# BradenDKelly/MetropolisMonteCarlo

Hardware: AMD Instinct MI355X
Metric: MC trial moves/sec (whole node), SPC/E NVT full Ewald fp64 (higher is better)
Workload: dtype f64

## Files before the change

metropolismontecarlo_amd/csrc/mmc_batch.inc:

```

#include <atomic>
#include <chrono>
#include <cmath>
#include <thread>
#include "mmc_state.hpp"
#include "mmc_solute_chain.hpp"

#define MMC_MAX_GROUPS 64
#define MMC_SERVER_AUTO_MAX 256
#define MMC_GEN_MAX 16
#define MMC_GEN_RING (MMC_GEN_MAX + 2)
#define MMC_QUEUE_STRIDE 32

#define MMC_CAND_EVERY 8
struct BatchCand {
    int enabled = 1;
    int skin_milli = 2000;
    bool tried = false;
    int state = 4;
    CandView v{};
    void *block = nullptr;
    int64_t bytes = 0;
    uint32_t t_build = 0;
    uint32_t d_refresh = 0;
    uint64_t epoch = ~0ULL;
    bool dirty = true;
    int64_t refresh_launches = 0;
    struct Range { int64_t r0, nr; unsigned long long count; bool pending; };
    std::vector<Range> ranges;
};

struct BatchSolute {
    int n = 0;
    bool charged = false;
    double mol[3 * (SOL_MAX_SITES + 1)] = { 0 };
    double charge[SOL_MAX_SITES] = { 0 }, eps[3 * SOL_MAX_SITES] = { 0 }, sig[3 * SOL_MAX_SITES] = { 0 };
    double q2 = 0.0;
    uint64_t hash = 0;
    double *d_par = nullptr;
    PartOut *h_parts = nullptr, *d_parts = nullptr;
    SoluteView view() const { return SoluteView{ d_par, n, charged ? 1 : 0 }; }
};

struct mmc_batch {
    DeviceSystem sys;
    BatchCand cand;
    BatchSolute sol;
    double lj_rcut = 0, qq_rcut = 0;
    int n_parts = 1;
    int kernel = 3;
    int server_wgs = -1;
    int wave_wgs = 0;
    int n_cus = 256;
    bool fast_ok = false;
    bool rigid_only = true;
    int image_by_molecule = -1;
    int zero_copy_moves = 0;
    MoveRec *h_moves[2] = { nullptr, nullptr };
    MoveRec *hd_moves[2] = { nullptr, nullptr };
    MoveRec *d_moves[2] = { nullptr, nullptr };
    PartOut *h_parts = nullptr, *d_parts = nullptr;
    int32_t *h_accept = nullptr, *d_accept = nullptr;
    int32_t *dev_accept = nullptr;
    int buf = 0;
    bool has_prev = false;
    std::vector<uint8_t> s_cur;
    std::vector<double> h_com, h_at;
    bool mirror_valid = false;
    int device_moves = 0;
    MoveRec *d_ring = nullptr;
    int ring_slots = MMC_GEN_RING;
    double *d_quat = nullptr;
    unsigned stamp = 0;
    int64_t steps_done = 0;
    int eval_parts = 0;
    int quat_mode = 0;
    double db[9] = { 0 };
    int persistent = -1;
    unsigned long long *h_ctrl = nullptr, *hd_ctrl = nullptr;
    unsigned long long *bar_ctrl = nullptr;
    int32_t *h_timeout = nullptr, *hd_timeout = nullptr;
    hipStream_t run_streams[MMC_MAX_GROUPS] = {};
    hipEvent_t run_events[MMC_MAX_GROUPS][2] = {};
    void *pool = nullptr;
    void (*pool_destroy)(void *) = nullptr;
    int steps_per_launch = 0;
    int whole_call = 0;
    int accept_on_device = -1;
    DecideConsts *d_decide = nullptr;
    DecideConsts decide_host{};
    std::vector<double> temps;
    double *d_temps = nullptr;
    unsigned *d_queue = nullptr;
    unsigned queue_base[MMC_MAX_GROUPS] = {};
    bool queue_reset = false;
    int server_stall_ms = 0;
    int64_t server_seq_offset = 0;
    bool needs_reload = false;
    std::vector<uint8_t> reloaded;
    int inject_torn = 0;
    bool vol_outstanding = false;
    bool vol_saved_fast_ok = false;
    int vol_saved_kernel = 0;
    std::vector<int32_t> pb_moved;
    int64_t trace_steps = 0;
    std::vector<double> trace_delta;
    std::vector<uint8_t> trace_flags;
    uint8_t *h_flags = nullptr, *hd_flags = nullptr, *d_flags = nullptr;
    uint8_t *bar_flags = nullptr;
    double2 *h_steps = nullptr, *hd_steps = nullptr, *d_steps = nullptr;
    void *obs_buf = nullptr;
    size_t obs_bytes = 0;
    void *obs_host = nullptr;
    size_t obs_host_bytes = 0;
    int coulomb_style = MMC_COULOMB_EWALD;
    bool s_stale = false;
    int local_stage = 1;
    int bond_chunk = 0;
    int ring_chunk = 0;
    int voronoi_prune = 1;
    uint64_t topology = 0;
    int state_chunk = 0;
    int state_delivery = -1;
    void *st_h[2] = { nullptr, nullptr }, *st_hd[2] = { nullptr, nullptr };
    void *st_d[2] = { nullptr, nullptr };
    size_t st_bytes = 0;
    hipEvent_t st_ev[2] = {};
    uint8_t *d_state_cur = nullptr;

// ... 515 lines not shown
                      b_cnt = up(2 * cqs * R), b_idx = up(2 * (int64_t)MMC_CAND_CAP * s.n_mol * R);
        const int64_t total = b_stat + b_d + b_q0 + b_cnt + b_idx;
        size_t free_b = 0, total_b = 0;
        void *blk = nullptr;
        if (hipMemGetInfo(&free_b, &total_b) == hipSuccess
            && (size_t)total + std::max<size_t>(total_b / 16, (size_t)1 << 30) <= free_b
            && hipMalloc(&blk, (size_t)total) == hipSuccess) {
            s.allocs.push_back(blk);
            char *p = (char *)blk;
            c.v.stat = (unsigned long long *)p; p += b_stat;
            c.v.D = (uint32_t *)p; p += b_d;
            c.v.q0 = (uint16_t *)p; p += b_q0;
            c.v.cnt = (uint16_t *)p; p += b_cnt;
            c.v.idx = (uint16_t *)p;
            c.block = blk;
            c.bytes = total;
            MMC_HIP(hipMemsetAsync(blk, 0, (size_t)(total - b_idx), s.stream));
            c.dirty = true;
        } else {
            (void)hipGetLastError();
            c.state = 2;
        }
    }
    if (!c.v.idx)
        return MMC_OK;
    const double gate_sq = std::max(pp.lj_gate_sq, pp.qq_gate_sq), gate = std::sqrt(gate_sq);
    const double wide = gate + 1e-3 * c.skin_milli;
    const uint32_t t_build = com_quant_gate(wide * wide, s.box);
    const uint32_t budget = cand_budget(t_build, com_quant_gate(gate_sq, s.box));
    if (t_build != c.t_build || budget != c.v.budget) {
        c.t_build = t_build;
        c.v.budget = budget;
        c.dirty = true;
    }
    c.d_refresh = (uint32_t)(((uint64_t)budget * 3 / 4) * ((uint64_t)budget * 3 / 4));
    c.state = budget > 0 ? 1 : 3;
    if (c.dirty || c.epoch != s.comq_epoch) {
        MMC_HIP(hipMemsetAsync(c.v.D, 0xff, sizeof(uint32_t) * (size_t)s.R, s.stream));
        MMC_HIP(hipStreamSynchronize(s.stream));
        c.dirty = false;
        c.epoch = s.comq_epoch;
        for (BatchCand::Range &g : c.ranges)
            g.pending = true;
    }
    return MMC_OK;
}

static int32_t batch_cand_stale(mmc_batch *b, hipStream_t stream, int64_t r0, int64_t nr)
{
    if (b->cand.v.idx) {
        MMC_HIP(hipMemsetAsync(b->cand.v.D + r0, 0xff, sizeof(uint32_t) * (size_t)nr, stream));
        for (BatchCand::Range &g : b->cand.ranges)
            if (g.r0 < r0 + nr && r0 < g.r0 + g.nr)
                g.pending = true;
    }
    return MMC_OK;
}

static int32_t batch_cand_for_launch(mmc_batch *b, hipStream_t stream, int64_t r0, int64_t nr, CandView *out)
{
    BatchCand &c = b->cand;
    *out = CandView{};
    if (!c.enabled || !c.v.idx || c.v.budget == 0)
        return batch_cand_stale(b, stream, r0, nr);
    BatchCand::Range *g = nullptr;
    for (BatchCand::Range &x : c.ranges)
        if (x.r0 == r0 && x.nr == nr)
            g = &x;
    if (!g) {
        c.ranges.push_back(BatchCand::Range{ r0, nr, 0ULL, true });
        g = &c.ranges.back();
    }
    if (g->pending || g->count % MMC_CAND_EVERY == 0) {
        k_cand_refresh<<<(unsigned)nr, 256, 0, stream>>>(b->sys.bv, c.v, (int)r0, c.t_build, c.d_refresh);
        MMC_HIP(hipGetLastError());
        c.refresh_launches++;
        g->pending = false;
    }
    g->count++;
    *out = c.v;
    return MMC_OK;
}

struct WaveForm { bool subst, img, multi, wolf, ladder; };

static int32_t batch_launch(mmc_batch *b, hipStream_t stream, int64_t r0, int64_t nr, int P, int kernel,
                            int buf, bool has_prev, const PairParams &pp,
                            hipEvent_t before_kernel = nullptr, const DevGen *dg = nullptr,
                            unsigned stamp = 0, const DevDecide *dd = nullptr)
{
    DeviceSystem &s = b->sys;
    const MoveRec *cur, *prev;
    const uint8_t *flagv = nullptr;
    if (dg) {
        flagv = b->hd_flags;
        const double2 *stp = b->hd_steps;
        if (!b->zero_copy_moves) {
            if (dd ? dd->fetch_flags : !b->bar_flags)
                k_fetch_bytes<<<(unsigned)((nr + 1023) / 1024), 256, 0, stream>>>(
                    b->d_flags + r0, b->hd_flags + r0, (int)nr);
            if (dg->upload_steps)
                MMC_HIP(hipMemcpyAsync(b->d_steps + r0, b->h_steps + r0, sizeof(double2) * nr,
                                       hipMemcpyHostToDevice, stream));
            flagv = b->bar_flags && !dd ? b->bar_flags : b->d_flags;
            stp = b->d_steps;
        }
        if (dg->n_gen > 0) {
            GenArgs ga;
            ga.steps = stp; ga.seed = dg->seed; ga.replica0 = dg->replica0;
            ga.rng_off = dg->rng_off; ga.step0 = dg->step; ga.n_gen = dg->n_gen;
            ga.ring = b->ring_slots; ga.ring_stride = s.R; ga.flag0 = flagv;
            ga.quat_mode = b->quat_mode;
            memcpy(ga.db, b->db, sizeof(ga.db));
            const int64_t n = nr * dg->n_gen;
            if (s.pb.on)
                k_propose<<<(unsigned)((n + 63) / 64), 64, 0, stream>>>(s.bv, s.rec, b->d_ring, ga, (int)r0,
                                                                        (int)nr, has_prev ? 1 : 0, s.pb_view());
            else
                k_propose<<<(unsigned)((n + 63) / 64), 64, 0, stream>>>(s.bv, s.rec, b->d_ring, ga,
                                                                        (int)r0, (int)nr, has_prev ? 1 : 0);
        }
        cur = batch_ring_slot(b, dg->step);
        prev = has_prev ? batch_ring_slot(b, dg->step + b->ring_slots - 1) : nullptr;
    } else {
        b->rigid_only = false;
        s.r_mol_max = INFINITY;
        if (!b->zero_copy_moves)
            MMC_HIP(hipMemcpyAsync(b->d_moves[buf] + r0, b->h_moves[buf] + r0,
                                   sizeof(MoveRec) * nr, hipMemcpyHostToDevice, stream));
        cur = b->dev_moves(buf);
        prev = has_prev ? b->dev_moves(buf ^ 1) : nullptr;
    }
    if (before_kernel)
        MMC_HIP(hipEventRecord(before_kernel, stream));
    if (b->sol.n)
        k_solute_move<<<(unsigned)((nr + SOLC_BLOCK / 16 - 1) / (SOLC_BLOCK / 16)), SOLC_BLOCK, 0, stream>>>(
            b->sol.view(), cur, s.qq_tab, s.fc, pp, s.box, b->sol.d_parts, (int)r0, (int)nr, stamp);
    dim3 grid((unsigned)P, (unsigned)nr);
    MMC_REQUIRE(!dd || (dg && P == 1 && !b->zero_copy_moves && kernel == 2), MMC_ERR_ASSERT,
                "the kernel's own accept decision needs device-side proposals, one part per move and the wave kernel");
    const bool wolf = b->coulomb_style == MMC_COULOMB_WOLF;
    if (kernel != 2)
        MMC_TRY(batch_cand_stale(b, stream, r0, nr));
    MMC_REQUIRE(!wolf || (kernel != 4 && !s.pb.on), MMC_ERR_ASSERT, "Wolf style reached a kernel without a Wolf form");
    using Yes = std::true_type;
    using No = std::false_type;
    if (kernel == 4) {
        MMC_REQUIRE(lat_applies(4 * P, (int)s.n_mol, (int)s.nkvecs), MMC_ERR_UNSUPPORTED,
                    "kernel 4 needs 4..%d parts (a multiple of 4) with at most %d molecules per pair "
                    "part", LAT_MAX_PARTS, LAT_MAXMOL);
        k_move_eval_lat<<<grid, LAT_WAVES * 64, 0, stream>>>(s.bv, s.rec, s.qq_tab, s.kpack, s.fc,
                                                             cur, prev, b->d_parts, 4 * P, pp, (int)r0,
                                                             flagv, stamp);
    } else if (kernel == 2) {
        const int64_t n_units = nr * P;
        int64_t wgs = (n_units + WV_MWAVES - 1) / WV_MWAVES;
        const int64_t cap = b->wave_wgs > 0 ? b->wave_wgs
                                            : (int64_t)(4 * (wolf ? WV_OCC_WOLF : WV_OCC) / WV_MWAVES) * b->n_cus;
        if (wgs > cap) wgs = cap;
        const bool img = dg && b->rigid_only && b->image_by_molecule != 0 &&
                         s.image_by_molecule(std::max(pp.lj_gate_sq, pp.qq_gate_sq)) &&
                         s.pairs_inside_slack(pp.qq_gate_sq, pp.qq_slack_sq) &&
                         s.pairs_inside_slack(pp.lj_gate_sq, pp.lj_slack_sq);
        const WaveForm f{ P != 1, img, dd && dd->n_sub > 1, wolf, dd && !b->temps.empty() };
        CandView cvv{};
        if (P == 1)
            MMC_TRY(batch_cand_for_launch(b, stream, r0, nr, &cvv));
        else
            MMC_TRY(batch_cand_stale(b, stream, r0, nr));
        auto launch = [&](auto subst, auto img_, auto multi, auto wolf_, auto ladder) {
            k_move_eval_wave<subst(), img_(), multi(), wolf_(), ladder()><<<(unsigned)wgs, WV_MWAVES * 64, 0, stream>>>(
                s.bv, s.rec, s.qq_tab, s.kpack, s.fc, cur, prev, dd ? dd->parts : b->d_parts, P, pp,
                (int)r0, (int)n_units, flagv, stamp, dd ? dd->dc : nullptr, dd ? (long long)dd->step : 0LL,
                dd ? dd->n_sub : 1, (int)(dg ? dg->step % b->ring_slots : 0), dd ? dd->queue : nullptr,
                dd ? dd->queue_base : 0u, cvv);
        };
        auto pick = [&](auto subst, auto img_, auto multi) {
            if (f.ladder) {
                if constexpr (!subst()) {
                    if (f.wolf) launch(subst, img_, multi, Yes{}, Yes{});
                    else launch(subst, img_, multi, No{}, Yes{});
                }
            } else if (f.wolf) launch(subst, img_, multi, Yes{}, No{});
            else launch(subst, img_, multi, No{}, No{});
        };
        if (f.multi) {
            if (f.img) pick(No{}, Yes{}, Yes{}); else pick(No{}, No{}, Yes{});
        } else if (!f.subst) {
            if (f.img) pick(No{}, Yes{}, No{}); else pick(No{}, No{}, No{});
        } else {
            if (f.img) pick(Yes{}, Yes{}, No{}); else pick(Yes{}, No{}, No{});
        }
    } else if (kernel == 1) {
        auto launch = [&](auto wolf_, const double *qq_tab, auto... per_box) {
            k_move_eval_fast<wolf_()><<<grid, MMC_BLOCK, 0, stream>>>(s.bv, s.rec, qq_tab, s.kpack, s.fc, cur, prev,
                                                                     b->d_parts, P, pp, (int)r0, flagv, stamp,
                                                                     per_box...);
        };
        if (s.pb.on) launch(No{}, nullptr, s.pb_view());
        else if (wolf) launch(Yes{}, s.qq_tab);
        else launch(No{}, s.qq_tab);
    } else {
        auto launch = [&](auto wolf_) {
            k_move_eval<wolf_()><<<grid, MMC_BLOCK, 0, stream>>>(s.bv, cur, prev, b->d_parts, P, pp, (int)r0,
                                                                 s.rec, flagv, stamp);
        };
        if (wolf) launch(Yes{}); else launch(No{});
    }
    MMC_HIP(hipGetLastError());
    return MMC_OK;
}

static int batch_server_parts(int64_t n_mol, int64_t R)
{
    int64_t pairs = (n_mol + 63) / 64;
    const int64_t cap = R == 1 ? 4 : SRV_WAVES - 1;
    if (pairs > cap) pairs = cap;
    if (pairs < 1) pairs = 1;
    return (int)pairs + 1;
}

static bool batch_server_applies(const mmc_batch *b)
{
    return b->fast_ok && b->kernel != 0 && b->device_moves && !b->quat_mode
           && b->sys.R <= (int64_t)b->n_cus;
}

static int batch_lat_shape(const mmc_batch *b)
{
    const DeviceSystem &s = b->sys;
    int G = b->server_wgs;
    if (G < 0)
        G = s.R * 4 <= (int64_t)b->n_cus ? 4 : 2;
    while (G >= 2 && !lat_applies(4 * G, (int)s.n_mol, (int)s.nkvecs))
        G--;
    if (G < 2 && b->server_wgs < 0) {
        G = (int)(((s.n_mol + LAT_MAXMOL - 1) / LAT_MAXMOL + 3 + LAT_WAVES - 1) / LAT_WAVES);
        while (G <= LAT_MAX_PARTS / LAT_WAVES && !lat_applies(4 * G, (int)s.n_mol, (int)s.nkvecs))
            G++;
        if (G > LAT_MAX_PARTS / LAT_WAVES)
            G = 0;
    }
    if (G < 2 || s.R * G > (int64_t)b->n_cus)
        return 0;
    return G;
}

static void batch_ctrl_clear(mmc_batch *b)
{
    memset(b->h_ctrl, 0, sizeof(unsigned long long) * b->sys.R);
    if (b->bar_ctrl) {
        for (int64_t r = 0; r < b->sys.R; r++)
            ((volatile unsigned long long *)b->bar_ctrl)[r] = 0ULL;
        mmc_bar_flush();
    }
}

static int32_t batch_server_start(mmc_batch *b, hipStream_t stream, int waves, const PairParams &pp,
// ... 443 lines not shown
```

metropolismontecarlo_amd/csrc/mmc_wave.hpp:

```cpp
#pragma once
#include "mmc_fast.hpp"
#include "mmc_propose.hpp"

#ifndef WV_WAVES
#define WV_WAVES 4
#endif
#ifndef WV_OCC
#define WV_OCC 5
#endif
#ifndef WV_OCC_WOLF
#define WV_OCC_WOLF 4
#endif
#ifndef WV_MWAVES
#define WV_MWAVES WV_WAVES
#endif
#ifndef WV_LIST
#define WV_LIST 640
#endif
#ifndef WV_PF
#define WV_PF 6
#endif
#define MMC_CQ_PAD (4 * 64 * (2 * WV_PF + 2))
#ifndef WV_TPF
#define WV_TPF 3
// ... 109 lines not shown
    return __builtin_amdgcn_readlane(v, src);
}

__device__ __forceinline__ double uniform_f64(double v)
{
    const long long b = __double_as_longlong(v);
    unsigned lo, hi;
    asm volatile("v_readfirstlane_b32 %0, %1" : "=s"(lo) : "v"((int)b));
    asm volatile("v_readfirstlane_b32 %0, %1" : "=s"(hi) : "v"((int)(b >> 32)));
    return __longlong_as_double((long long)(((unsigned long long)hi << 32) | lo));
}

__device__ __forceinline__ double lane_f64(double v, int src)
{
    const long long b = __double_as_longlong(v);
    const unsigned lo = (unsigned)__builtin_amdgcn_readlane((int)b, src);
    const unsigned hi = (unsigned)__builtin_amdgcn_readlane((int)(b >> 32), src);
    return __longlong_as_double((long long)(((unsigned long long)hi << 32) | lo));
}

__device__ __forceinline__ unsigned long long wave_shfl_xor_u64(unsigned long long v, int m)
{
    const unsigned lo = (unsigned)__shfl_xor((int)(unsigned)v, m, 64);
    const unsigned hi = (unsigned)__shfl_xor((int)(unsigned)(v >> 32), m, 64);
    return ((unsigned long long)hi << 32) | lo;
}
__device__ __forceinline__ unsigned long long wave_min_u64(unsigned long long v)
{
#pragma unroll
    for (int m = 32; m > 0; m >>= 1) {
        const unsigned long long o = wave_shfl_xor_u64(v, m);
        v = o < v ? o : v;
    }
    return v;
}

__device__ __forceinline__ void phase_row_moderate(double x, double L, cplx *row )
{
    double sn, cs;
    sincos_moderate(MMC_TWOPI * x / L, sn, cs);
    const cplx e1 = { cs, sn }, one = { 1.0, 0.0 };
    row[5] = one;
    row[6] = e1;
    row[4] = c_conj(e1);
    cplx p = e1;
#pragma unroll
    for (int k = 2; k <= 5; k++) {
        p = c_mul(p, e1);
        row[5 + k] = p;
        row[5 - k] = c_conj(p);
    }
}

template <bool LADDER = false>
__device__ __forceinline__ int wave_decide(const double *outw, bool ov_old, bool ov_new,
                                           const DecideConsts *__restrict__ dc, long long step, int r,
                                           int scur, int lane, double *delta_out = nullptr, bool store_flags = true,
                                           bool flip_s = true)
{
    const double delta = mmc_move_delta(outw, ov_old, ov_new, dc->factor);
    if (delta_out)
        *delta_out = delta;
    const double x = delta / (LADDER ? dc->temps[r] : dc->temperature);
    const double u = mmc_metropolis_uniform(ChainKey{ dc->seed, dc->replica0 + (uint32_t)r }, (uint64_t)step);
    bool met;
    if (x < 0.0) met = true;
    else if (1.0 - x > u + 1e-9) met = true;
    else if ((1.0 + x) * u > 1.0 + 1e-9) met = false;
    else met = exp(-x) > u;
    const int acc = (met && !(ov_old || ov_new)) ? 1 : 0;
    if (store_flags && lane == 0)
        dc->flags[r] = (uint8_t)(acc | ((scur ^ (flip_s ? acc : 0)) << 1));
    return acc;
}

__device__ __forceinline__ int wave_ticket(unsigned *queue, unsigned base, int n_waves, int lane)
{
    unsigned t = 0;
    if (lane == 0)
        t = atomicAdd(queue, 1u);
    return n_waves + (int)(__builtin_amdgcn_readfirstlane(t) - base);
}

template <bool SUBST, bool IMG, bool MULTI = false, bool WOLF = false, bool LADDER = false>
__global__ __launch_bounds__(WV_MWAVES * 64)
__attribute__((amdgpu_waves_per_eu(WOLF ? WV_OCC_WOLF : WV_OCC, WOLF ? WV_OCC_WOLF : WV_OCC))) void k_move_eval_wave(
    BatchView bv, double *rec, const double *__restrict__ qq_tab,
    const int32_t *__restrict__ kpack, FastConsts fc, const MoveRec *__restrict__ cur,
    const MoveRec *__restrict__ prev, PartOut *out, int n_parts, PairParams pp, int r_base,
    int n_units, const uint8_t *flagv, unsigned stamp, const DecideConsts *__restrict__ dc, long long dec_step,
    int n_sub_arg, int slot0, unsigned *queue, unsigned queue_base, CandView cv)
{
    const int n_sub = MULTI ? n_sub_arg : 1;
    const bool cand_on = !SUBST && cv.idx != nullptr;
    __shared__ __align__(16) WaveSharedT<WV_MWAVES, !WOLF> sm;
    const int tid = threadIdx.x, lane0 = tid & 63;
    const int wv = __builtin_amdgcn_readfirstlane(tid >> 6);

    for (int k = tid; k < MMC_QQ_TABLE_DOUBLES; k += WV_MWAVES * 64)
        sm.qtab[k] = qq_tab[k];
    __syncthreads();

    const int n_mol = bv.n_mol, nkv = bv.nkvecs;
    const double box = bv.box;
    const BoxConsts bc = box_consts(box);
    const int np = WOLF ? n_parts : (n_parts == 1) ? 1 : n_parts - 1;
    const int plen = (n_mol + np - 1) / np;
    const bool same_gate = pp.lj_gate_sq == pp.qq_gate_sq;
    const double inv_box = uniform_f64(1.0 / box);
    uint32_t gate_q;
    asm volatile("v_readfirstlane_b32 %0, %1" : "=s"(gate_q) : "v"(com_quant_gate(fmax(pp.lj_gate_sq, pp.qq_gate_sq), box)));
    wv_list_t *const list = sm.list[wv];
    const double *const pvw = sm.pvw[wv];

    for (int unit = blockIdx.x * WV_MWAVES + wv; unit < n_units;
         unit = MULTI && queue ? wave_ticket(queue, queue_base, gridDim.x * WV_MWAVES, lane0)
                               : unit + gridDim.x * WV_MWAVES) {
        int lane = lane0;
        if (!MULTI)
            asm volatile("" : "+v"(lane));
        int rl = unit, part = 0;
        if (n_parts != 1) {
            rl = unit / n_parts;
            part = unit - rl * n_parts;
        }
        const int r = r_base + rl;
        const bool do_pairs = WOLF ? true : (n_parts == 1) || (part < n_parts - 1);
        const bool do_recip = WOLF ? false : (n_parts == 1) || (part == n_parts - 1);
        const int j_begin = do_pairs ? min(part * plen, n_mol) : 0;
        const int j_end = do_pairs ? min(j_begin + plen, n_mol) : 0;
        double *const myrec = rec + (int64_t)r * n_mol * MMC_RSTRIDE;

        int flags_carry = -1;
        double e_sum = 0.0;
        unsigned acc_mask = 0, ovl_mask = 0, kind_mask = 0;
        uint32_t d_cur = MMC_CAND_STALE;
        unsigned n_cand = 0;
        if (!SUBST && cand_on)
            d_cur = (uint32_t)__builtin_amdgcn_readfirstlane((int)cv.D[r]);
      for (int sub = 0; sub < n_sub; sub++) {
        if (MULTI) {
            lane = lane0;
            asm volatile("" : "+v"(lane));
        }
        const MoveRec *cur_s = cur, *prev_s = prev;
        if (n_sub > 1) {
            const int sl = (slot0 + sub) % dc->ring_slots, slp = (slot0 + sub + dc->ring_slots - 1) % dc->ring_slots;
            cur_s = dc->ring + (int64_t)sl * dc->ring_stride;
            if (sub > 0)
                prev_s = dc->ring + (int64_t)slp * dc->ring_stride;
        }
        WV_STAMP(0);
        const double *mvp = reinterpret_cast<const double *>(cur_s + r);
        double w = 0.0;
        if (lane < MV_Q_NEW)
            w = mvp[lane];
        WV_STAMP(1);
        const int gflag = flags_carry >= 0 ? flags_carry : (flagv ? __builtin_amdgcn_readfirstlane((int)flagv[r]) : -1);
        const long long hdr = __double_as_longlong(w);
        const int i0 = lane_i32((int)hdr, 0) - 1;
        const int flags = gflag >= 0 ? gflag : lane_i32((int)(hdr >> 32), 0);
        const bool commit = prev_s && (flags & 1);
        const int scur = (flags >> 1) & 1;

        int pend = -1;
        uint32_t pcxy = 0, pcz = 0;
        if (commit) {
            const double *pvp = reinterpret_cast<const double *>(prev_s + r);
            double pw = 0.0;
            if (lane < 9) pw = pvp[MV_AT_NEW + lane];
            else if (lane < 12) pw = pvp[MV_COM_NEW + lane - 9];
            else if (lane == 12) pw = pvp[0];
            else if (lane < 17) pw = pvp[MV_Q_NEW + lane - 13];
            pend = lane_i32((int)__double_as_longlong(pw), 12) - 1;
            if (lane < 12)
                sm.pvw[wv][lane] = pw;
            if (part == 0 && lane < 12) {
                myrec[(int64_t)pend * MMC_RSTRIDE + lane] = pw;
                if (lane < 9) {
                    const int a = lane / 3, d = lane % 3;
                    (d == 0 ? bv.ax : d == 1 ? bv.ay : bv.az)[r * bv.atom_stride + 3 * pend + a] = pw;
                } else {
                    const int d = lane - 9;
                    (d == 0 ? bv.comx : d == 1 ? bv.comy : bv.comz)[r * bv.mol_stride + pend] = pw;
                    comq_store(bv, r, pend, d, pw, inv_box);
                }
            }
            if (!SUBST && cand_on) {
                const int cq = (lane >= 9 && lane < 12) ? (int)com_quant(pw, inv_box) : 0;
                pcxy = (uint32_t)lane_i32(cq, 9) | (uint32_t)lane_i32(cq, 10) << 16;
                pcz = (uint32_t)lane_i32(cq, 11);
            }
            if (bv.quat) {
                const double q0 = wave_pick(pw, 13), q1 = wave_pick(pw, 14),
                             q2 = wave_pick(pw, 15), q3 = wave_pick(pw, 16);
                if (part == 0 && lane >= 13 && lane < 17)
                    quat_commit(bv, r, pend, lane - 13, pw, q0 * q0 + q1 * q1 + q2 * q2 + q3 * q3 > 0.25);
            }
            wave_sync();
            if (WOLF && !SUBST)
                asm volatile("s_waitcnt vmcnt(0)" ::: "memory");
        }

#define WV_CQ_BASE (bv.comq + (int64_t)r * 3 * bv.cq_stride)
#define WV_PART_DST (out + (int64_t)r * n_parts + part)
        auto decide_here = [&](bool o0, bool o1) -> int {
            if (!dc)
                return 0;
            if (n_sub <= 1)
                return wave_decide<LADDER>(sm.outw[wv], o0, o1, dc, dec_step, r, scur, lane, nullptr, true, !WOLF);
            double delta;
            const bool last = sub + 1 == n_sub;
            const int acc = wave_decide<LADDER>(sm.outw[wv], o0, o1, dc, dec_step + sub, r, scur, lane, &delta, last, !WOLF);
            if (acc) {
                e_sum += delta;
                acc_mask |= 1u << sub;
            }
            if (o0 || o1)
                ovl_mask |= 1u << sub;
            kind_mask |= (unsigned)((lane_i32((int)(hdr >> 32), 0) >> 8) & 1) << sub;
            flags_carry = acc | ((scur ^ (WOLF ? 0 : acc)) << 1);
            if (last) {
                wave_sync();
                if (lane < 7)
                    sm.outw[wv][lane] = lane == 0 ? e_sum
                                 : lane == 1 ? __longlong_as_double((long long)acc_mask | ((long long)ovl_mask << 32))
                                 : lane == 2 ? __longlong_as_double((long long)kind_mask) : 0.0;
                wave_sync();
            }
            return acc;
        };
#define WV_DECIDE(o0, o1) decide_here(o0, o1)
#define WV_RECORD_OVL(o) (n_sub > 1 ? false : (o))
#define WV_STORE_IF (sub + 1 == n_sub)
#define WV_STORE_SYSTEM MULTI
#define WV_ZERO opaque_f64(0.0)
#define WV_SUBST SUBST
#define WV_IMG IMG
#define WV_WOLF WOLF
#define WV_VIRIAL (!MULTI)
#ifndef WV_XY_MOVE
#define WV_XY_MOVE 1
#endif
#define WV_XY WV_XY_MOVE
#define WV_PASSES 2
#ifndef WV_ONE_CALL_MOVE
#define WV_ONE_CALL_MOVE 1
#endif
#define WV_ONE_CALL WV_ONE_CALL_MOVE
#define WV_CAND (!SUBST)
#define WV_AFTER_PHASE_TABLES                                                                    \
    if (!SUBST && commit)                                                                        \
        asm volatile("s_waitcnt vmcnt(0)" ::: "memory");
#include "mmc_wave_unit.inc"
#undef WV_AFTER_PHASE_TABLES
#undef WV_IMG
#undef WV_WOLF
#undef WV_VIRIAL
#undef WV_PASSES
#undef WV_ONE_CALL
#undef WV_CAND
#undef WV_XY
#undef WV_SUBST
#undef WV_ZERO
#undef WV_CQ_BASE
#undef WV_PART_DST
#undef WV_DECIDE
#undef WV_RECORD_OVL
#undef WV_STORE_IF
#undef WV_STORE_SYSTEM
        if (n_sub > 1)
            asm volatile("s_waitcnt vmcnt(0)" ::: "memory");
      }
        if (!SUBST && cand_on && lane == 0) {
            atomicAdd(cv.stat + (int64_t)r * MMC_CAND_STATS, (unsigned long long)n_cand);
            atomicAdd(cv.stat + (int64_t)r * MMC_CAND_STATS + 1, (unsigned long long)((unsigned)n_sub - n_cand));
        }
    }
}

struct TotalWaveShared {
    alignas(16) double qtab[MMC_QQ_TABLE_DOUBLES];
    int32_t list[WV_WAVES][WV_LIST];
};

#define WV_TOTAL_WAVES_PER_SIMD 5
template <bool COHERENT, bool IMG>
__device__ __forceinline__ void total_wave_body(
    TotalWaveShared &sm, const BatchView &bv, const double *__restrict__ rec,
    const double *__restrict__ qq_tab, const FastConsts &fc, const PairParams &pp, TotalPart *out,
    int units_per_rep, int n_units, int paired, int wg, int n_wgs, int j_chunk = 0)
{
    const int tid = threadIdx.x, lane0 = tid & 63;
    const int wv = __builtin_amdgcn_readfirstlane(tid >> 6);
    for (int k = tid; k < MMC_QQ_TABLE_DOUBLES; k += WV_WAVES * 64)
        sm.qtab[k] = qq_tab[k];
    __syncthreads();

    const int n_mol = bv.n_mol;
    const double box = bv.box;
    const BoxConsts bc = box_consts(box);
    const bool same_gate = pp.lj_gate_sq == pp.qq_gate_sq;
    const double inv_box = 1.0 / box;
    const uint32_t gate_q = com_quant_gate(fmax(pp.lj_gate_sq, pp.qq_gate_sq), box);
    int32_t *const list = sm.list[wv];

    for (int unit = wg * WV_WAVES + wv; unit < n_units; unit += n_wgs * WV_WAVES) {
        int lane = lane0;
        asm volatile("" : "+v"(lane));
        const int r = unit / units_per_rep, u = unit - r * units_per_rep;
        const double *myrec = rec + (int64_t)r * n_mol * MMC_RSTRIDE;
        const uint16_t *cq0 = bv.comq + (int64_t)r * 3 * bv.cq_stride;
        const uint32_t *sxy = reinterpret_cast<const uint32_t *>(cq0);
        const uint16_t *sz = cq0 + 2 * bv.cq_stride;
        double a_lj = 0, a_v = 0, a_q = 0;
        unsigned long long ovm = 0;

        const int n_ch = j_chunk > 0 ? (n_mol + j_chunk - 1) / j_chunk : 1;
        const int j_lo = j_chunk > 0 ? (u % n_ch) * j_chunk : 0;
        const int j_hi = j_chunk > 0 ? min(j_lo + j_chunk, n_mol) : n_mol;
        const int iA = j_chunk > 0 ? u / n_ch : u, iB = n_mol - 1 - u;
        const bool hasB = paired && iB > iA;
        double wAB = 0.0;
        if (lane < MMC_REC)
            wAB = myrec[(int64_t)iA * MMC_RSTRIDE + lane];
        else if (hasB && lane >= 16 && lane < 16 + MMC_REC)
            wAB = myrec[(int64_t)iB * MMC_RSTRIDE + lane - 16];

        auto process = [&](int cnt) {
            wave_sync();
            for (int n0 = 0; n0 < cnt; n0 += 64) {
                const int n = n0 + lane;
                const bool act = n < cnt;
                const int ent = act ? list[n] : 0;
                const int j = ent & ((1 << 27) - 1);
                const bool isB = (ent >> 27) != 0;
                double t[MMC_REC];
                const double2 *src = reinterpret_cast<const double2 *>(myrec + (int64_t)j * MMC_RSTRIDE);
#pragma unroll
                for (int q = 0; q < 6; q++) {
                    const double2 v = src[q];
                    t[2 * q] = v.x;
                    t[2 * q + 1] = v.y;
                }
                const int own0 = isB ? 16 : 0;
                auto mine = [&](int word) { return wave_pick(wAB, own0 + word); };
                const double ccx = mine(9), ccy = mine(10), ccz = mine(11);
                double m[3] = { 0, 0, 0 };
                auto min1 = [&](int d, double a, double b) {
                    if constexpr (IMG)
                        return fma(m[d], bc.neg, b - a);
                    else
                        return vector1D_abs(a, b, bc);
                };
                if constexpr (IMG) {
                    const double dx = t[9] - ccx, dy = t[10] - ccy, dz = t[11] - ccz;
                    m[0] = (fabs(dx) < bc.half) ? 0.0 : copysign(1.0, dx);
// ... 364 lines not shown
```

metropolismontecarlo_amd/csrc/mmc_wave_unit.inc:

```
#ifndef WV_NS
#define WV_NS 2
#define WV_NS_DEFAULTED
#endif
#if WV_NS == 2
#define WV_IF2(...) __VA_ARGS__
#else
#define WV_IF2(...)
#endif
#ifndef WV_SUBST
#define WV_SUBST 1
#define WV_SUBST_DEFAULTED
#endif
#ifndef WV_IMG
#define WV_IMG 0
#define WV_IMG_DEFAULTED
#endif
#ifndef WV_PASSES
#define WV_PASSES 1
#define WV_PASSES_DEFAULTED
#endif
#ifndef WV_ONE_CALL
#define WV_ONE_CALL 0
#define WV_ONE_CALL_DEFAULTED
#endif
#ifndef WV_XY
#define WV_XY 0
#define WV_XY_DEFAULTED
#endif
#ifndef WV_KPF
#define WV_KPF 2
#endif
#ifndef WV_WOLF
#define WV_WOLF 0
#define WV_WOLF_DEFAULTED
#endif
#ifndef WV_ZERO
#define WV_ZERO 0.0
#define WV_ZERO_DEFAULTED
#endif
#ifndef WV_VIRIAL
#define WV_VIRIAL 1
#define WV_VIRIAL_DEFAULTED
#endif
#ifndef WV_STORE_IF
#define WV_STORE_IF true
#define WV_STORE_IF_DEFAULTED
#endif
#if WV_NS != 2
static_assert(WV_VIRIAL, "the one-state body always delivers the virial");
#endif
        double *const outw = sm.outw[wv];
        unsigned long long ovm0 = 0, ovm1 = 0;

        constexpr bool wv_wolf = WV_WOLF;
        if constexpr (!wv_wolf) {
        if (do_recip) {
            {
                const int t = lane < 18 ? lane : 0;
                const int st = t / 9, q = t - 9 * st;
                const double x = wave_pick(w, (st ? MV_AT_NEW : MV_AT_OLD) + q);
                if (lane < 18)
                    phase_row_moderate(x, box, sm.ptab[wv][st][q / 3][q % 3]);
            }
            wave_sync();
            WV_STAMP(2);
#ifdef WV_AFTER_PHASE_TABLES
            WV_AFTER_PHASE_TABLES
#endif
        }
        auto recip_loop = [&]() {
            double a_rec = 0;
#ifdef WV_S_BASE
            const double *So = WV_S_BASE;
            double *Sn = WV_S_DST;
#else
            const double *So = s_buf(bv, r, scur);
            double *Sn = s_buf(bv, r, scur ^ 1);
#endif
            int kcs[WV_KPF], kps[WV_KPF];
            double cfs[WV_KPF];
            double2 sos[WV_KPF];
#pragma unroll
            for (int q = 0; q < WV_KPF; q++) {
                kcs[q] = min(lane + 64 * q, nkv - 1);
                kps[q] = kpack[kcs[q]];
                cfs[q] = bv.cfac[kcs[q]];
                sos[q] = *reinterpret_cast<const double2 *>(So + 2 * kcs[q]);
            }
#if WV_XY
            const int colp = kpack[MMC_NK_STRIDE + lane];
#endif
#if WV_XY
            cplx xyp[2][3];
            {
                const int cx = colp & 15, cy = (colp >> 4) & 15;
#pragma unroll
                for (int st = 0; st < 2; st++)
#pragma unroll
                    for (int l = 0; l < 3; l++)
                        xyp[st][l] = c_mul_fused(sm.ptab[wv][st][l][0][5 + cx], sm.ptab[wv][st][l][1][cy]);
            }
#endif
#ifdef WV_S_MIRROR
            unsigned long long s_sum = 0;
#endif
            const int n_it = (nkv + 63) >> 6;
            int k = lane;
            for (int it = 0; it < n_it; it++) {
                const int kc = kcs[0], kp = kps[0];
                const double cf = cfs[0];
                const double2 so = sos[0];
#pragma unroll
                for (int q = 0; q + 1 < WV_KPF; q++) {
                    kcs[q] = kcs[q + 1]; kps[q] = kps[q + 1]; cfs[q] = cfs[q + 1]; sos[q] = sos[q + 1];
                }
                kcs[WV_KPF - 1] = min(k + 64 * WV_KPF, nkv - 1);
                kps[WV_KPF - 1] = kpack[kcs[WV_KPF - 1]];
                cfs[WV_KPF - 1] = bv.cfac[kcs[WV_KPF - 1]];
                sos[WV_KPF - 1] = *reinterpret_cast<const double2 *>(So + 2 * kcs[WV_KPF - 1]);
                {
                    const int kz = (kp >> 8) & 15;
                    double nr = so.x, ni = so.y;
#if WV_XY
                    const int col = (kp >> 12) & (MMC_KCOLS - 1);
                    auto from_col = [&](const cplx &v) {
                        cplx o;
                        o.re = wave_pick(v.re, col);
                        o.im = wave_pick(v.im, col);
                        return o;
                    };
#else
                    const int kx = kp & 15, ky = (kp >> 4) & 15;
#endif
#pragma unroll
                    for (int l = 0; l < 3; l++) {
#if WV_XY
                        const cplx tn = c_mul_fused(from_col(xyp[1][l]), sm.ptab[wv][1][l][2][kz]);
                        const cplx to = c_mul_fused(from_col(xyp[0][l]), sm.ptab[wv][0][l][2][kz]);
#else
                        const cplx tn = c_mul_fused(c_mul_fused(sm.ptab[wv][1][l][0][5 + kx], sm.ptab[wv][1][l][1][ky]),
                                                sm.ptab[wv][1][l][2][kz]);
                        const cplx to = c_mul_fused(c_mul_fused(sm.ptab[wv][0][l][0][5 + kx], sm.ptab[wv][0][l][1][ky]),
                                                sm.ptab[wv][0][l][2][kz]);
#endif
                        nr = fma(fc.q[l], tn.re - to.re, nr);
                        ni = fma(fc.q[l], tn.im - to.im, ni);
                    }
                    *reinterpret_cast<double2 *>(Sn + 2 * kc) = make_double2(nr, ni);
#ifdef WV_S_MIRROR
                    {
                        typedef double s_piece __attribute__((ext_vector_type(2)));
                        s_piece v;
                        v.x = nr; v.y = ni;
                        double *mp = WV_S_MIRROR + 2 * kc;
                        asm volatile("global_store_dwordx4 %0, %1, off sc0 sc1" ::"v"(mp), "v"(v) : "memory");
                        if (k < nkv)
                            s_sum += (unsigned long long)__double_as_longlong(nr)
                                     + 3ULL * (unsigned long long)__double_as_longlong(ni);
                    }
#endif
                    const double wgt = k < nkv ? cf : 0.0;
                    a_rec = fma(wgt, fma(nr, nr, ni * ni) - fma(so.x, so.x, so.y * so.y), a_rec);
                }
                k += 64;
            }
            wave_sum1_store(a_rec, &outw[6], outw, lane);
#ifdef WV_S_MIRROR
            s_sum = wave_sum_u64(s_sum);
            if (lane == 0)
                sm.pvw[wv][0] = __longlong_as_double((long long)s_sum);
#endif
            WV_STAMP(3);
            wave_sync();
        };
        if (do_recip)
            recip_loop();
        }
        if (!do_recip && lane == 0)
            outw[6] = WV_ZERO;

        if (do_pairs) {
            if (lane < 6)
                outw[lane] = WV_ZERO;
            double cc[2][3];
            uint32_t cqxy[2], cqz[2];
            {
                const bool is_com = WV_IF2((lane >= MV_COM_OLD && lane < MV_COM_OLD + 3) ||)
                                    (lane >= MV_COM_NEW && lane < MV_COM_NEW + 3);
                const int myq = is_com ? (int)com_quant(w, inv_box) : 0;
#pragma unroll
                for (int d = 0; d < 3; d++) {
                    WV_IF2(cc[0][d] = lane_f64(w, MV_COM_OLD + d);)
                    cc[1][d] = lane_f64(w, MV_COM_NEW + d);
                }
                WV_IF2(cqxy[0] = (uint32_t)lane_i32(myq, MV_COM_OLD) | (uint32_t)lane_i32(myq, MV_COM_OLD + 1) << 16;)
                cqxy[1] = (uint32_t)lane_i32(myq, MV_COM_NEW) | (uint32_t)lane_i32(myq, MV_COM_NEW + 1) << 16;
                WV_IF2(cqz[0] = (uint32_t)lane_i32(myq, MV_COM_OLD + 2);)
                cqz[1] = (uint32_t)lane_i32(myq, MV_COM_NEW + 2);
            }

            auto process = [&](int cnt) {
                WV_IF2(double a_lj0 = 0, a_v0 = 0, a_q0 = 0;)
                double a_lj1 = 0, a_v1 = 0, a_q1 = 0;
                wave_sync();
                for (int n0 = 0; n0 < cnt; n0 += 64) {
                    const int n = n0 + lane;
                    const int j = n < cnt ? list[n] : 0;
                    const bool act = (n < cnt) && (j != i0);
                    double t[MMC_REC];
                    const double2 *src = reinterpret_cast<const double2 *>(myrec + (int64_t)j * MMC_RSTRIDE);
#pragma unroll
                    for (int q = 0; q < 6; q++) {
                        const double2 v = src[q];
                        t[2 * q] = v.x;
                        t[2 * q + 1] = v.y;
                    }
                    if (n0 == 0)
                        WV_STAMP(5);
                    if (WV_SUBST && j == pend) {
#pragma unroll
                        for (int q = 0; q < MMC_REC; q++)
                            t[q] = pvw[q];
                    }
                    WV_IF2(bool g0, l0;)
                    bool g1, l1;
                    constexpr bool wv_img = WV_IMG;
                    constexpr bool wv_virial = WV_VIRIAL;
                    double m[2][3] = { { 0, 0, 0 }, { 0, 0, 0 } };
                    auto min1 = [&](int st, int d, double a, double b) {
                        if constexpr (wv_img)
                            return fma(m[st][d], bc.neg, b - a);
                        else
                            return vector1D_abs(a, b, bc);
                    };
#define WV_MIN1(st, d, a, b) min1(st, d, a, b)
                    {
                        if constexpr (wv_img) {
#pragma unroll
                            for (int d = 0; d < 3; d++) {
                                const double d1 = t[9 + d] - cc[1][d];
                                m[1][d] = (fabs(d1) < bc.half) ? 0.0 : copysign(1.0, d1);
#if WV_NS == 2
                                const double d0 = t[9 + d] - cc[0][d];
                                m[0][d] = (fabs(d0) < bc.half) ? 0.0 : copysign(1.0, d0);
#endif
                            }
                        }
#if WV_NS == 2
                        const double x0 = WV_MIN1(0, 0, cc[0][0], t[9]), y0 = WV_MIN1(0, 1, cc[0][1], t[10]),
                                     z0 = WV_MIN1(0, 2, cc[0][2], t[11]);
                        const double c0 = x0 * x0 + y0 * y0 + z0 * z0;
                        g0 = act && (c0 < pp.qq_gate_sq);
                        l0 = same_gate ? g0 : (act && (c0 < pp.lj_gate_sq));
#endif
                        const double x1 = WV_MIN1(1, 0, cc[1][0], t[9]), y1 = WV_MIN1(1, 1, cc[1][1], t[10]),
                                     z1 = WV_MIN1(1, 2, cc[1][2], t[11]);
                        const double c1 = x1 * x1 + y1 * y1 + z1 * z1;
                        g1 = act && (c1 < pp.qq_gate_sq);
                        l1 = same_gate ? g1 : (act && (c1 < pp.lj_gate_sq));
                    }
                    WV_IF2(const unsigned long long gm0 = wave_ballot(g0);)
                    const unsigned long long gm1 = wave_ballot(g1);
#if WV_PASSES == 2
#define WV_PAIR_FENCE
                    auto pass = [&](auto stc, bool l, unsigned long long gm, unsigned long long &ovm,
                                    double &a_lj, double &a_v, double &a_q) {
                        constexpr int ST = decltype(stc)::value;
                        auto atoms = [&](auto exc, uint32_t &umin) {
                        constexpr bool EXACT = decltype(exc)::value;
#pragma unroll 1
                        for (int a = 0; a < 3; a++) {
                            const int base_w = (ST ? MV_AT_NEW : MV_AT_OLD) + 3 * a;
                            const double ax = lane_f64(w, base_w), ay = lane_f64(w, base_w + 1),
                                         az = lane_f64(w, base_w + 2);
                            auto pair1 = [&](int ab, double bx, double by, double bz) {
                                const double qq = fc.qq9[ab];
                                const double px = WV_MIN1(ST, 0, ax, bx), py = WV_MIN1(ST, 1, ay, by),
                                             pz = WV_MIN1(ST, 2, az, bz);
                                const double u = px * px + py * py + pz * pz;
                                const unsigned long long km = (wv_img ? ~0ULL : wave_ballot(u < pp.qq_slack_sq)) & gm;
                                if constexpr (EXACT) {
                                    const bool qneg = (fc.qneg_mask >> ab) & 1;
                                    const unsigned long long cm = wave_ballot(u < pp.ovr) & gm;
                                    const unsigned long long qm = qneg ? cm : 0ULL, cold = cm & ~qm;
// ... 256 lines not shown
                        list[cnt + lanes_below(m)] = j;
                    cnt += __popcll(m & m_end);
                    base += 64;
                }
                pxy += 256 * WV_PF;
                pz += 128 * WV_PF;
#if WV_ONE_CALL
            }
#ifdef WV_CAND
            }
            cand_pre = false;
#endif
            WV_STAMP(4);
            if (cnt)
                process(cnt);
            }
#else
                if (cnt > WV_LIST - 64 * WV_PF) {
                    process(cnt);
                    cnt = 0;
                }
            }
            WV_STAMP(4);
            if (cnt)
                process(cnt);
#endif
            WV_STAMP(6);
        } else if (lane < 6) {
            outw[lane] = WV_ZERO;
        }
#ifdef WV_S_MIRROR
        if (do_recip && !do_pairs) {
            wave_sync();
            if (lane == 0)
                outw[0] = sm.pvw[wv][0];
        }
#endif

#ifdef WV_UNIT_NO_STORE
        if (lane == 0)
            outw[7] = __longlong_as_double((long long)((ovm0 != 0ULL ? 1 : 0) | (ovm1 != 0ULL ? 2 : 0)));
#else
        wave_sync();
        {
#ifdef WV_DECIDE
            const int accept = WV_DECIDE(ovm0 != 0ULL, ovm1 != 0ULL);
#else
            const int accept = 0;
#endif
            if (WV_STORE_IF) {
                const uint32_t csum = part_checksum_lanes(lane < 7 ? outw[lane] : 0.0, lane, stamp);
#ifdef WV_RECORD_OVL
                if (lane == 0)
                    outw[7] = pack_ovl(WV_RECORD_OVL(ovm0 != 0ULL), WV_RECORD_OVL(ovm1 != 0ULL), stamp, csum, accept);
#else
                if (lane == 0)
                    outw[7] = pack_ovl(ovm0 != 0ULL, ovm1 != 0ULL, stamp, csum, accept);
#endif
            }
        }
        wave_sync();
#ifdef WV_STORE_WT
        store_part<true>(WV_PART_DST, sm.outw[wv], lane);
#else
#ifndef WV_STORE_SYSTEM
#define WV_STORE_SYSTEM false
#define WV_STORE_SYSTEM_DEFAULTED
#endif
        if (WV_STORE_IF)
            store_part<WV_STORE_SYSTEM>(WV_PART_DST, sm.outw[wv], lane);
#ifdef WV_STORE_SYSTEM_DEFAULTED
#undef WV_STORE_SYSTEM
#undef WV_STORE_SYSTEM_DEFAULTED
#endif
#endif
        wave_sync();
        WV_STAMP(7);
#endif
#ifdef WV_STORE_IF_DEFAULTED
#undef WV_STORE_IF
#undef WV_STORE_IF_DEFAULTED
#endif
#undef WV_IF2
#ifdef WV_XY_DEFAULTED
#undef WV_XY
#undef WV_XY_DEFAULTED
#endif
#ifdef WV_ONE_CALL_DEFAULTED
#undef WV_ONE_CALL
#undef WV_ONE_CALL_DEFAULTED
#endif
#ifdef WV_PASSES_DEFAULTED
#undef WV_PASSES
#undef WV_PASSES_DEFAULTED
#endif
#ifdef WV_IMG_DEFAULTED
#undef WV_IMG
#undef WV_IMG_DEFAULTED
#endif
#ifdef WV_SUBST_DEFAULTED
#undef WV_SUBST
#undef WV_SUBST_DEFAULTED
#endif
#ifdef WV_ZERO_DEFAULTED
#undef WV_ZERO
#undef WV_ZERO_DEFAULTED
#endif
#ifdef WV_VIRIAL_DEFAULTED
#undef WV_VIRIAL
#undef WV_VIRIAL_DEFAULTED
#endif
#ifdef WV_WOLF_DEFAULTED
#undef WV_WOLF
#undef WV_WOLF_DEFAULTED
#endif
#ifdef WV_NS_DEFAULTED
#undef WV_NS
#undef WV_NS_DEFAULTED
#endif
```

Before: 157.3 million.

## Pass wave kernel arguments via cached device struct and reload per phase

Packs the wave kernel's large by-value arguments (BatchView, PairParams, CandView, FastConsts, box constants, pointers) into a device-resident WaveArgs struct. The struct is cached in a small host-managed ring and uploaded only when its contents change. Inside the kernel the fields are re-read from constant address space at the start of each phase instead of staying live across the whole kernel. The aim is to cut scalar register pressure and kernarg size. In exchange, uploads force a synchronize on all streams, and each phase pays extra scalar loads.

```diff
diff --git a/metropolismontecarlo_amd/csrc/mmc_batch.inc b/metropolismontecarlo_amd/csrc/mmc_batch.inc
--- a/metropolismontecarlo_amd/csrc/mmc_batch.inc
+++ b/metropolismontecarlo_amd/csrc/mmc_batch.inc
@@ -2,6 +2,7 @@
 #include <atomic>
 #include <chrono>
 #include <cmath>
+#include <mutex>
 #include <thread>
 #include "mmc_state.hpp"
 #include "mmc_solute_chain.hpp"
@@ -30,6 +31,15 @@
     std::vector<Range> ranges;
 };
 
+#define MMC_WAVE_ARG_SLOTS 4
+struct BatchWaveArgs {
+    WaveArgs *d = nullptr;
+    WaveArgs h[MMC_WAVE_ARG_SLOTS];
+    int n = 0, next = 0;
+    int64_t uploads = 0;
+    std::mutex m;
+};
+
 struct BatchSolute {
     int n = 0;
     bool charged = false;
@@ -45,6 +55,7 @@
 struct mmc_batch {
     DeviceSystem sys;
     BatchCand cand;
+    BatchWaveArgs wargs;
     BatchSolute sol;
     double lj_rcut = 0, qq_rcut = 0;
     int n_parts = 1;
@@ -726,6 +737,31 @@
     return MMC_OK;
 }
 
+static int32_t batch_wave_args(mmc_batch *b, const WaveArgs &w, const WaveArgs **out)
+{
+    BatchWaveArgs &c = b->wargs;
+    std::lock_guard<std::mutex> lk(c.m);
+    if (!c.d)
+        MMC_TRY(b->sys.dmalloc((void **)&c.d, sizeof(WaveArgs) * MMC_WAVE_ARG_SLOTS));
+    for (int k = 0; k < c.n; k++)
+        if (memcmp(&c.h[k], &w, sizeof(w)) == 0) {
+            *out = c.d + k;
+            return MMC_OK;
+        }
+    MMC_HIP(hipStreamSynchronize(b->sys.stream));
+    for (hipStream_t st : b->run_streams)
+        if (st)
+            MMC_HIP(hipStreamSynchronize(st));
+    const int k = c.next;
+    MMC_HIP(hipMemcpy(c.d + k, &w, sizeof(w), hipMemcpyHostToDevice));
+    memcpy(&c.h[k], &w, sizeof(w));
+    c.next = (k + 1) % MMC_WAVE_ARG_SLOTS;
+    c.n = std::max(c.n, k + 1);
+    c.uploads++;
+    *out = c.d + k;
+    return MMC_OK;
+}
+
 struct WaveForm { bool subst, img, multi, wolf, ladder; };
 
 static int32_t batch_launch(mmc_batch *b, hipStream_t stream, int64_t r0, int64_t nr, int P, int kernel,
@@ -812,12 +848,19 @@
             MMC_TRY(batch_cand_for_launch(b, stream, r0, nr, &cvv));
         else
             MMC_TRY(batch_cand_stale(b, stream, r0, nr));
+        WaveArgs w;
+        memset(&w, 0, sizeof(w));
+        w.bv = s.bv; w.pp = pp; w.cv = cvv; w.fc = s.fc;
+        w.bc.half = 0.5 * s.bv.box; w.bc.neg = -s.bv.box; w.bc.box = s.bv.box;
+        w.rec = s.rec; w.qq_tab = s.qq_tab; w.kpack = s.kpack;
+        const WaveArgs *wa = nullptr;
+        MMC_TRY(batch_wave_args(b, w, &wa));
         auto launch = [&](auto subst, auto img_, auto multi, auto wolf_, auto ladder) {
             k_move_eval_wave<subst(), img_(), multi(), wolf_(), ladder()><<<(unsigned)wgs, WV_MWAVES * 64, 0, stream>>>(
-                s.bv, s.rec, s.qq_tab, s.kpack, s.fc, cur, prev, dd ? dd->parts : b->d_parts, P, pp,
+                wa, cur, prev, dd ? dd->parts : b->d_parts, P,
                 (int)r0, (int)n_units, flagv, stamp, dd ? dd->dc : nullptr, dd ? (long long)dd->step : 0LL,
                 dd ? dd->n_sub : 1, (int)(dg ? dg->step % b->ring_slots : 0), dd ? dd->queue : nullptr,
-                dd ? dd->queue_base : 0u, cvv);
+                dd ? dd->queue_base : 0u);
         };
         auto pick = [&](auto subst, auto img_, auto multi) {
             if (f.ladder) {
diff --git a/metropolismontecarlo_amd/csrc/mmc_wave.hpp b/metropolismontecarlo_amd/csrc/mmc_wave.hpp
--- a/metropolismontecarlo_amd/csrc/mmc_wave.hpp
+++ b/metropolismontecarlo_amd/csrc/mmc_wave.hpp
@@ -215,34 +215,97 @@
     return n_waves + (int)(__builtin_amdgcn_readfirstlane(t) - base);
 }
 
+struct WaveArgs {
+    BatchView bv;
+    PairParams pp;
+    CandView cv;
+    FastConsts fc;
+    BoxConsts bc;
+    double *rec;
+    const double *qq_tab;
+    const int32_t *kpack;
+};
+typedef const WaveArgs __attribute__((address_space(4))) *wave_args_k;
+struct WaveFcView {
+    const double __attribute__((address_space(4))) *qq9, *eps9, *sig9;
+    double q[3];
+    int32_t qneg_mask, lj_mask;
+};
+__device__ __forceinline__ wave_args_k wave_args_phase(const WaveArgs *p)
+{
+    asm volatile("" : "+s"(p));
+    return (wave_args_k)p;
+}
+template <class T> __device__ __forceinline__ T wave_args_copy(const void __attribute__((address_space(4))) *src)
+{
+    static_assert(sizeof(T) % 8 == 0, "whole 8-byte words");
+    union { T v; uint64_t w[sizeof(T) / 8]; } u;
+    const uint64_t __attribute__((address_space(4))) *s = (const uint64_t __attribute__((address_space(4))) *)src;
+#pragma unroll
+    for (unsigned k = 0; k < sizeof(T) / 8; k++)
+        u.w[k] = s[k];
+    return u.v;
+}
+__device__ __forceinline__ BatchView wave_args_copy(const BatchView __attribute__((address_space(4))) &s)
+{
+    BatchView d;
+    d.comx = s.comx; d.comy = s.comy; d.comz = s.comz; d.ax = s.ax; d.ay = s.ay; d.az = s.az;
+    d.mol_stride = s.mol_stride; d.atom_stride = s.atom_stride;
+    d.first0 = s.first0; d.cnt = s.cnt; d.atype = s.atype; d.charge = s.charge; d.eps = s.eps; d.sig = s.sig;
+    d.n_mol = s.n_mol; d.n_atoms = s.n_atoms; d.n_types = s.n_types; d.box = s.box;
+    d.S = s.S; d.nk_stride = s.nk_stride; d.kxyz = s.kxyz; d.cfac = s.cfac; d.kmap = s.kmap;
+    d.nkvecs = s.nkvecs; d.nk = s.nk; d.kappa = s.kappa; d.factor = s.factor;
+    d.comq = s.comq; d.cq_stride = s.cq_stride; d.quat = s.quat;
+    return d;
+}
+__device__ __forceinline__ CandView wave_args_copy(const CandView __attribute__((address_space(4))) &s)
+{
+    CandView d;
+    d.idx = s.idx; d.cnt = s.cnt; d.q0 = s.q0; d.D = s.D; d.stat = s.stat; d.budget = s.budget;
+    return d;
+}
+#define WV_ARGS_PHASE                                                                                  \
+    const wave_args_k wq = wave_args_phase(wa);                                                        \
+    [[maybe_unused]] const BatchView bv = wave_args_copy(wq->bv);                                      \
+    [[maybe_unused]] const PairParams pp = wave_args_copy<PairParams>(&wq->pp);                        \
+    [[maybe_unused]] const CandView cv = wave_args_copy(wq->cv);                                       \
+    [[maybe_unused]] const BoxConsts bc = wave_args_copy<BoxConsts>(&wq->bc);                          \
+    [[maybe_unused]] const WaveFcView fc = { wq->fc.qq9, wq->fc.eps9, wq->fc.sig9,                     \
+                                             { wq->fc.q[0], wq->fc.q[1], wq->fc.q[2] },                \
+                                             wq->fc.qneg_mask, wq->fc.lj_mask };                       \
+    [[maybe_unused]] const int n_mol = bv.n_mol, nkv = bv.nkvecs;                                      \
+    [[maybe_unused]] const double box = bv.box;                                                        \
+    [[maybe_unused]] const bool same_gate = pp.lj_gate_sq == pp.qq_gate_sq;                            \
+    [[maybe_unused]] const int32_t *const kpack = (const int32_t *)wq->kpack;                          \
+    [[maybe_unused]] double *const myrec = (double *)wq->rec + (int64_t)r * bv.n_mol * MMC_RSTRIDE;
+
 template <bool SUBST, bool IMG, bool MULTI = false, bool WOLF = false, bool LADDER = false>
 __global__ __launch_bounds__(WV_MWAVES * 64)
 __attribute__((amdgpu_waves_per_eu(WOLF ? WV_OCC_WOLF : WV_OCC, WOLF ? WV_OCC_WOLF : WV_OCC))) void k_move_eval_wave(
-    BatchView bv, double *rec, const double *__restrict__ qq_tab,
-    const int32_t *__restrict__ kpack, FastConsts fc, const MoveRec *__restrict__ cur,
-    const MoveRec *__restrict__ prev, PartOut *out, int n_parts, PairParams pp, int r_base,
+    const WaveArgs *__restrict__ wa, const MoveRec *__restrict__ cur,
+    const MoveRec *__restrict__ prev, PartOut *out, int n_parts, int r_base,
     int n_units, const uint8_t *flagv, unsigned stamp, const DecideConsts *__restrict__ dc, long long dec_step,
-    int n_sub_arg, int slot0, unsigned *queue, unsigned queue_base, CandView cv)
+    int n_sub_arg, int slot0, unsigned *queue, unsigned queue_base)
 {
     const int n_sub = MULTI ? n_sub_arg : 1;
-    const bool cand_on = !SUBST && cv.idx != nullptr;
+    const wave_args_k wa0 = (wave_args_k)wa;
+    const bool cand_on = !SUBST && wa0->cv.idx != nullptr;
     __shared__ __align__(16) WaveSharedT<WV_MWAVES, !WOLF> sm;
     const int tid = threadIdx.x, lane0 = tid & 63;
     const int wv = __builtin_amdgcn_readfirstlane(tid >> 6);
 
-    for (int k = tid; k < MMC_QQ_TABLE_DOUBLES; k += WV_MWAVES * 64)
-        sm.qtab[k] = qq_tab[k];
+    {
+        const double *qq_tab = (const double *)wa0->qq_tab;
+        for (int k = tid; k < MMC_QQ_TABLE_DOUBLES; k += WV_MWAVES * 64)
+            sm.qtab[k] = qq_tab[k];
+    }
     __syncthreads();
 
-    const int n_mol = bv.n_mol, nkv = bv.nkvecs;
-    const double box = bv.box;
-    const BoxConsts bc = box_consts(box);
     const int np = WOLF ? n_parts : (n_parts == 1) ? 1 : n_parts - 1;
-    const int plen = (n_mol + np - 1) / np;
-    const bool same_gate = pp.lj_gate_sq == pp.qq_gate_sq;
-    const double inv_box = uniform_f64(1.0 / box);
+    const int plen = (wa0->bv.n_mol + np - 1) / np;
+    const double inv_box = uniform_f64(1.0 / wa0->bv.box);
     uint32_t gate_q;
-    asm volatile("v_readfirstlane_b32 %0, %1" : "=s"(gate_q) : "v"(com_quant_gate(fmax(pp.lj_gate_sq, pp.qq_gate_sq), box)));
+    asm volatile("v_readfirstlane_b32 %0, %1" : "=s"(gate_q) : "v"(com_quant_gate(fmax(wa0->pp.lj_gate_sq, wa0->pp.qq_gate_sq), wa0->bv.box)));
     wv_list_t *const list = sm.list[wv];
     const double *const pvw = sm.pvw[wv];
 
@@ -260,17 +323,22 @@
         const int r = r_base + rl;
         const bool do_pairs = WOLF ? true : (n_parts == 1) || (part < n_parts - 1);
         const bool do_recip = WOLF ? false : (n_parts == 1) || (part == n_parts - 1);
-        const int j_begin = do_pairs ? min(part * plen, n_mol) : 0;
-        const int j_end = do_pairs ? min(j_begin + plen, n_mol) : 0;
-        double *const myrec = rec + (int64_t)r * n_mol * MMC_RSTRIDE;
+        int j_begin = 0, j_end = 0;
 
         int flags_carry = -1;
         double e_sum = 0.0;
         unsigned acc_mask = 0, ovl_mask = 0, kind_mask = 0;
         uint32_t d_cur = MMC_CAND_STALE;
         unsigned n_cand = 0;
-        if (!SUBST && cand_on)
-            d_cur = (uint32_t)__builtin_amdgcn_readfirstlane((int)cv.D[r]);
+        {
+            WV_ARGS_PHASE
+            if (do_pairs) {
+                j_begin = min(part * plen, n_mol);
+                j_end = min(j_begin + plen, n_mol);
+            }
+            if (!SUBST && cand_on)
+                d_cur = (uint32_t)__builtin_amdgcn_readfirstlane((int)cv.D[r]);
+        }
       for (int sub = 0; sub < n_sub; sub++) {
         if (MULTI) {
             lane = lane0;
@@ -299,6 +367,7 @@
         int pend = -1;
         uint32_t pcxy = 0, pcz = 0;
         if (commit) {
+            WV_ARGS_PHASE
             const double *pvp = reinterpret_cast<const double *>(prev_s + r);
             double pw = 0.0;
             if (lane < 9) pw = pvp[MV_AT_NEW + lane];
@@ -382,6 +451,7 @@
 #endif
 #define WV_ONE_CALL WV_ONE_CALL_MOVE
 #define WV_CAND (!SUBST)
+#define WV_PHASE_ARGS WV_ARGS_PHASE
 #define WV_AFTER_PHASE_TABLES                                                                    \
     if (!SUBST && commit)                                                                        \
         asm volatile("s_waitcnt vmcnt(0)" ::: "memory");
@@ -393,6 +463,7 @@
 #undef WV_PASSES
 #undef WV_ONE_CALL
 #undef WV_CAND
+#undef WV_PHASE_ARGS
 #undef WV_XY
 #undef WV_SUBST
 #undef WV_ZERO
@@ -406,6 +477,7 @@
             asm volatile("s_waitcnt vmcnt(0)" ::: "memory");
       }
         if (!SUBST && cand_on && lane == 0) {
+            WV_ARGS_PHASE
             atomicAdd(cv.stat + (int64_t)r * MMC_CAND_STATS, (unsigned long long)n_cand);
             atomicAdd(cv.stat + (int64_t)r * MMC_CAND_STATS + 1, (unsigned long long)((unsigned)n_sub - n_cand));
         }
diff --git a/metropolismontecarlo_amd/csrc/mmc_wave_unit.inc b/metropolismontecarlo_amd/csrc/mmc_wave_unit.inc
--- a/metropolismontecarlo_amd/csrc/mmc_wave_unit.inc
+++ b/metropolismontecarlo_amd/csrc/mmc_wave_unit.inc
@@ -45,6 +45,10 @@
 #ifndef WV_STORE_IF
 #define WV_STORE_IF true
 #define WV_STORE_IF_DEFAULTED
+#endif
+#ifndef WV_PHASE_ARGS
+#define WV_PHASE_ARGS
+#define WV_PHASE_ARGS_DEFAULTED
 #endif
 #if WV_NS != 2
 static_assert(WV_VIRIAL, "the one-state body always delivers the virial");
@@ -54,6 +58,7 @@
 
         constexpr bool wv_wolf = WV_WOLF;
         if constexpr (!wv_wolf) {
+        WV_PHASE_ARGS
         if (do_recip) {
             {
                 const int t = lane < 18 ? lane : 0;
@@ -180,6 +185,7 @@
             outw[6] = WV_ZERO;
 
         if (do_pairs) {
+            WV_PHASE_ARGS
             if (lane < 6)
                 outw[lane] = WV_ZERO;
             double cc[2][3];
@@ -200,6 +206,7 @@
             }
 
             auto process = [&](int cnt) {
+                WV_PHASE_ARGS
                 WV_IF2(double a_lj0 = 0, a_v0 = 0, a_q0 = 0;)
                 double a_lj1 = 0, a_v1 = 0, a_q1 = 0;
                 wave_sync();
@@ -622,6 +629,10 @@
 #undef WV_STORE_IF_DEFAULTED
 #endif
 #undef WV_IF2
+#ifdef WV_PHASE_ARGS_DEFAULTED
+#undef WV_PHASE_ARGS
+#undef WV_PHASE_ARGS_DEFAULTED
+#endif
 #ifdef WV_XY_DEFAULTED
 #undef WV_XY
 #undef WV_XY_DEFAULTED
```

Result: no change. 158.8 million (median of 6 runs) (+1.0%).
